# pkuyzy/TLC-GNN

Hardware: AMD Instinct MI355X
Metric: persistence-images/sec + LP-forward edges/sec, PubMed-scale, 1/2/4/8 GPU (higher is better)
Workload: dtype f64; 1 GPU

## Files before the change

### tlc-gnn_amd/csrc/pd_tiny.hip

```cpp
#include "tlc_common.h"
#include "tlc_kernels.h"

namespace {

template <typename T>
struct LaneArr {
    T* base;
    __device__ __forceinline__ T& operator[](int k) const { return base[k * 64]; }
};

struct LaneBytes8 {
    unsigned char* base;
    __device__ __forceinline__ unsigned char& operator[](int j) const { return base[(j >> 3) * 512 + (j & 7)]; }
};
struct LaneBytes8Slice {
    LaneBytes8 b;
    int off;
    __device__ __forceinline__ unsigned char& operator[](int j) const { return b[off + j]; }
};

__device__ __forceinline__ double tiny_key_asc(double fa, double fb) {
    const double hi = fa > fb ? fa : fb, lo = fa < fb ? fa : fb;
    return hi + (lo + 1.0) * 1e-6;
}
__device__ __forceinline__ double tiny_key_desc(double fa, double fb) {
    const double hi = fa > fb ? fa : fb, lo = fa < fb ? fa : fb;
    return lo - (101.0 - hi) * 1e-6;
}

__device__ __forceinline__ double tiny_norm_cdf(double x) {
    const double z = x * 0.70710678118654752440;
    const double t = z * z;
    double a = 4.22140728880708822e-18;
    a = fma(a, t, -8.03273501241577328e-17);
    a = fma(a, t, 1.44832646435981379e-15);
    a = fma(a, t, -2.46682701026445706e-14);
    a = fma(a, t, 3.95542951645852569e-13);
    a = fma(a, t, -5.94779401363763541e-12);
    a = fma(a, t, 8.35070279514723971e-11);
    a = fma(a, t, -1.08922210371485731e-09);
    a = fma(a, t, 1.31225329638028058e-08);
    a = fma(a, t, -1.45038522231504685e-07);
    a = fma(a, t, 1.45891690009337058e-06);
    a = fma(a, t, -1.32275132275132281e-05);
    a = fma(a, t, 1.06837606837606838e-04);
    a = fma(a, t, -7.57575757575757575e-04);
    a = fma(a, t, 4.62962962962962937e-03);
    a = fma(a, t, -2.38095238095238082e-02);
    a = fma(a, t, 1.00000000000000006e-01);
    a = fma(a, t, -3.33333333333333315e-01);
    a = fma(a, t, 1.0);
    return fma(0.5 * 1.1283791670955126, z * a, 0.5);
}

struct TinyImage {
    double px[25];
    __device__ __forceinline__ void clear() {
#pragma unroll
        for (int k = 0; k < 25; ++k) px[k] = 0.0;
    }
    __device__ __forceinline__ void add(double b, double d) {
        const double pers = d - b;
        const double wgt = pers < 0.0 ? 0.0 : (pers > 1.0 ? 1.0 : pers);
        if (wgt == 0.0) return;
        const double step = ((1.0 + 0.2) - 0.0) / 6.0;
        double cb[6], cp[6];
#pragma unroll
        for (int g = 0; g < 6; ++g) {
            cb[g] = tiny_norm_cdf((double)g * step - b);
            cp[g] = tiny_norm_cdf((double)g * step - pers);
        }
#pragma unroll
        for (int i = 0; i < 5; ++i) {
            const double db = cb[i + 1] - cb[i];
#pragma unroll
            for (int j = 0; j < 5; ++j) px[i * 5 + j] += wgt * (db * (cp[j + 1] - cp[j]));
        }
    }
};

constexpr int TN = TLC_T_NMAX, TM = TLC_T_MMAX;
constexpr int TP = TLC_T_NMAX + TLC_T_MMAX;
constexpr size_t T_OA = 0;
constexpr size_t T_OB = T_OA + (size_t)TM * 64 * 8;
constexpr size_t T_OC = T_OB + (size_t)TN * 64 * 8;
constexpr size_t T_OD = T_OC + (size_t)TN * 64 * 8;
constexpr size_t T_OE = T_OD + (size_t)TM * 64 * 2;
constexpr size_t TINY_WG_BYTES = T_OE + 5 * (size_t)TN * 64;
static_assert(2 * TP + 2 * TN <= TN * 8, "points + tree tables alias the second distance array (8 bytes per lane and row)");
static_assert(2 * (size_t)TM * 64 + (size_t)TN * 64 <= 5 * (size_t)TN * 64, "order / components / Pos-Neg list alias the tight-successor tables");

}

__device__ __forceinline__ void tiny_slot(const TlcPdParams p, unsigned char* lds, int lane, int slot) {
    LaneArr<double> ew{(double*)(lds + T_OA) + lane};
    const LaneArr<double>& key = ew;
    LaneArr<double> du{(double*)(lds + T_OB) + lane};
    const LaneArr<double>& f = du;
    LaneArr<double> dv{(double*)(lds + T_OC) + lane};
    const LaneArr<double>& dist = dv;
    LaneBytes8 cbytes{lds + T_OC + 8 * (size_t)lane};
    LaneBytes8Slice ptb{cbytes, 0};
    LaneBytes8Slice ptd{cbytes, TP};
    LaneBytes8Slice par{cbytes, 2 * TP};
    LaneBytes8Slice pedge{cbytes, 2 * TP + TN};
    LaneArr<unsigned short> eab{(unsigned short*)(lds + T_OD) + lane};
    LaneArr<unsigned char> cntU{lds + T_OE + lane};
    LaneArr<unsigned char> nxtU{lds + T_OE + (size_t)TN * 64 + lane};
    LaneArr<unsigned char> cntV{lds + T_OE + 2 * (size_t)TN * 64 + lane};
    LaneArr<unsigned char> nxtV{lds + T_OE + 3 * (size_t)TN * 64 + lane};
    LaneArr<unsigned char> ambl{lds + T_OE + 4 * (size_t)TN * 64 + lane};
    LaneArr<unsigned char> ord{lds + T_OE + lane};
    LaneArr<unsigned char> comp{lds + T_OE + (size_t)TM * 64 + lane};
    LaneArr<unsigned char> pn{lds + T_OE + (size_t)TM * 64 + (size_t)TN * 64 + lane};
    int npts = 0;
    int i, n, m2 = 0, lu, lv, m = 0;
    const unsigned* adir = nullptr;
    const double* alw = nullptr;
    {
        if (p.tiny_bin_list) {
            int s = slot, b = 0;
            while (b < TLC_TINY_BINS - 1 && s >= ((p.tiny_bin_cnt[b] + 63) >> 6)) { s -= (p.tiny_bin_cnt[b] + 63) >> 6; ++b; }
            const int wi = s * 64 + lane;
            if (wi >= p.tiny_bin_cnt[b]) return;
            i = p.tiny_bin_list[(size_t)b * p.tiny_bin_stride + wi];
        } else {
            int tier_count = p.tier_count;
            if (p.tier_count_dev) { const int c = *p.tier_count_dev; tier_count = c < tier_count ? c : tier_count; }
            const int wi = slot * 64 + lane;
            if (wi >= tier_count) return;
            i = p.tier_list[wi];
        }
        n = p.hdr_n[i]; m2 = p.hdr_m2[i]; lu = p.hdr_lu[i]; lv = p.hdr_lv[i];
        adir = p.small_dir ? p.small_dir + (size_t)i * (2 * TLC_S_MMAX) : p.A_dir + p.edge_off[i];
        alw = p.small_dir ? p.small_lw + (size_t)i * (2 * TLC_S_MMAX) : p.A_lw + p.edge_off[i];
    }
    int status = TLC_ST_OK;
    TinyImage img;
    img.clear();
    unsigned long long* pc = p.phase_cycles;
    unsigned long long t_prev = pc ? clock64() : 0ull;
#define TINY_STAMP(k) do { if (pc) { const unsigned long long _t = clock64(); if (lane == 0) atomicAdd(&pc[(k)], _t - t_prev); t_prev = _t; } } while (0)
    {
        for (int j0 = 0; j0 < m2; j0 += 8) {
            unsigned ee[8];
            double wq[8];
#pragma unroll
            for (int q = 0; q < 8; ++q) {
                const bool in = j0 + q < m2;
                ee[q] = in ? adir[j0 + q] : 0u;
                wq[q] = in ? alw[j0 + q] : 0.0;
            }
#pragma unroll
            for (int q = 0; q < 8; ++q) {
                const unsigned a = ee[q] >> 16, b = ee[q] & 0xffffu;
                if (j0 + q < m2 && a < b && m < TM) { eab[m] = (unsigned short)((a << 8) | b); ew[m] = wq[q]; ++m; }
            }
        }
    }
    TINY_STAMP(0);
    const double INF = __longlong_as_double(0x7FF0000000000000ll);
    auto bellman_ford_from = [&](int s, const LaneArr<double>& d) {
        for (int y = 0; y < n; ++y) d[y] = INF;
        d[s] = 0.0;
        for (int round = 0; round <= n; ++round) {
            bool ch = false;
            for (int e = 0; e < m; ++e) {
                const unsigned ab = eab[e];
                const int a = (int)(ab >> 8), b = (int)(ab & 0xffu);
                const double w = ew[e];
                const double da = d[a], db = d[b];
                const double ca = da + w, cb = db + w;
                if (ca < db) { d[b] = ca; ch = true; }
                if (cb < da) { d[a] = cb; ch = true; }
            }
            if (!ch) break;
        }
    };
    const bool far = lu < 0;
    if (far) {
        bellman_ford_from(0, dist);
        for (int y = 0; y < n; ++y) if (dist[y] == INF) status = TLC_ST_DISCONNECTED;
        if (status == TLC_ST_OK && n == 1) status = TLC_ST_NO_TREE_EDGE;
    } else {
        bellman_ford_from(lu, du);
        for (int y = 0; y < n; ++y) if (du[y] == INF) status = TLC_ST_DISCONNECTED;
        if (status == TLC_ST_OK) {
            bellman_ford_from(lv, dv);
            double dmx = 0.0;
            for (int y = 0; y < n; ++y) { const double a = du[y], b = dv[y]; dmx = a > dmx ? a : dmx; dmx = b > dmx ? b : dmx; cntU[y] = 0; cntV[y] = 0; }
            const double tol = 1e-10 * (1.0 + dmx);
            for (int e = 0; e < m; ++e) {
                const unsigned ab = eab[e];
                const int a = (int)(ab >> 8), b = (int)(ab & 0xffu);
                const double w = ew[e];
                const double ua = du[a], ub = du[b], va = dv[a], vb = dv[b];
                if (a != lu && (w + ub) - ua <= tol) { cntU[a] = (unsigned char)(cntU[a] + 1); nxtU[a] = (unsigned char)e; }
                if (b != lu && (w + ua) - ub <= tol) { cntU[b] = (unsigned char)(cntU[b] + 1); nxtU[b] = (unsigned char)e; }
                if (a != lv && (w + vb) - va <= tol) { cntV[a] = (unsigned char)(cntV[a] + 1); nxtV[a] = (unsigned char)e; }
                if (b != lv && (w + va) - vb <= tol) { cntV[b] = (unsigned char)(cntV[b] + 1); nxtV[b] = (unsigned char)e; }
            }
            double mx = 0.0;
            int namb = 0;
            for (int x = 0; x < n; ++x) {
                double fr = 0.0;
                if (x != lu && x != lv) {
                    double d1 = 0.0, d2 = 0.0;
                    bool amb = false;
                    int a = x, steps = 0;
                    while (a != lu) {
                        if (cntU[a] != 1 || ++steps > n) { amb = true; break; }
                        const int e = nxtU[a];
                        const unsigned ab = eab[e];
                        d1 = d1 + ew[e];
                        a = ((int)(ab >> 8) == a) ? (int)(ab & 0xffu) : (int)(ab >> 8);
                    }
                    a = x; steps = 0;
                    while (!amb && a != lv) {
                        if (cntV[a] != 1 || ++steps > n) { amb = true; break; }
                        const int e = nxtV[a];
                        const unsigned ab = eab[e];
                        d2 = d2 + ew[e];
                        a = ((int)(ab >> 8) == a) ? (int)(ab & 0xffu) : (int)(ab >> 8);
                    }
                    if (amb) ambl[namb++] = (unsigned char)x;
                    fr = d1 + d2;
                }
                f[x] = fr;
            }
            for (int q = 0; q < namb; ++q) {
                const int x = ambl[q];
                bellman_ford_from(x, dist);
                f[x] = dist[lu] + dist[lv];
            }
            if (namb && p.stats) atomicAdd(&p.stats[0], (unsigned long long)namb);
            for (int x = 0; x < n; ++x) { const double v = f[x]; mx = v > mx ? v : mx; }
            TINY_STAMP(1);
            if (mx == 0.0) status = TLC_ST_ZERO_RANGE;
            else for (int x = 0; x < n; ++x) f[x] = f[x] / mx;
        }
        if (status == TLC_ST_OK) {
            for (int e = 0; e < m; ++e) { const unsigned ab = eab[e]; key[e] = tiny_key_asc(f[ab >> 8], f[ab & 0xffu]); }
            for (int e = 0; e < m; ++e) {
                const double k = key[e];
                int r = 0;
                for (int e2 = 0; e2 < m; ++e2) { const double k2 = key[e2]; r += (k2 < k || (k2 == k && e2 < e)) ? 1 : 0; }
                ord[r] = (unsigned char)e;
            }
            auto find = [&](int x) {
                int c = comp[x];
                while (x != c) { const int g = comp[c]; comp[x] = (unsigned char)g; x = g; c = comp[x]; }
                return x;
            };
            for (int y = 0; y < n; ++y) comp[y] = (unsigned char)y;
            int imin = 0, imax = 0;
            {
                double fmin = f[0], fmax = f[0];
                for (int y = 1; y < n; ++y) { const double v = f[y]; if (v < fmin) { fmin = v; imin = y; } if (v > fmax) { fmax = v; imax = y; } }
            }
            for (int t = 0; t < m; ++t) {
                const unsigned ab = eab[ord[t]];
                const int a = (int)(ab >> 8), b = (int)(ab & 0xffu);
                const int pu = find(a), pv = find(b);
                if (pu != pv) {
                    const int small = (f[pu] <= f[pv]) ? pu : pv, large = pu + pv - small;
                    const int max_node = (f[a] > f[b]) ? a : b;
                    if (f[large] < f[max_node]) { ptb[npts] = (unsigned char)large; ptd[npts] = (unsigned char)max_node; ++npts; }
                    comp[large] = (unsigned char)small;
                }
            }
            TINY_STAMP(2);
            ptb[npts] = (unsigned char)imin; ptd[npts] = (unsigned char)imax; ++npts;
            for (int e = 0; e < m; ++e) { const unsigned ab = eab[e]; key[e] = tiny_key_desc(f[ab >> 8], f[ab & 0xffu]); }
            for (int e = 0; e < m; ++e) {
                const double k = key[e];
                int r = 0;
                for (int e2 = 0; e2 < m; ++e2) { const double k2 = key[e2]; r += (k2 > k || (k2 == k && e2 < e)) ? 1 : 0; }
                ord[r] = (unsigned char)e;
            }
            for (int y = 0; y < n; ++y) comp[y] = (unsigned char)y;
            int npos = 0, nneg = 0;
            for (int t = 0; t < m; ++t) {
                const int e = ord[t];
                const unsigned ab = eab[e];
                const int pu = find((int)(ab >> 8)), pv = find((int)(ab & 0xffu));
                if (pu != pv) {
                    pn[TM - 1 - nneg++] = (unsigned char)e;
                    const int small = (f[pu] <= f[pv]) ? pu : pv, large = pu + pv - small;
                    comp[small] = (unsigned char)large;
                } else {
                    pn[npos++] = (unsigned char)e;
                }
            }
            TINY_STAMP(3);
            if (nneg == 0) status = TLC_ST_NO_TREE_EDGE;
            else if (npos > 0) {
                for (int y = 0; y < n; ++y) par[y] = 0xFFu;
                const int root = (int)(eab[pn[TM - 1]] >> 8);
                par[root] = (unsigned char)root;
                for (int round = 0; round < n; ++round) {
                    bool ch = false;
                    for (int t = 0; t < nneg; ++t) {
                        const int e = pn[TM - 1 - t];
                        const unsigned ab = eab[e];
                        const int a = (int)(ab >> 8), b = (int)(ab & 0xffu);
                        const unsigned pa = par[a], pb = par[b];
                        if (pa != 0xFFu && pb == 0xFFu) { par[b] = (unsigned char)a; pedge[b] = (unsigned char)e; ch = true; }
                        else if (pb != 0xFFu && pa == 0xFFu) { par[a] = (unsigned char)b; pedge[a] = (unsigned char)e; ch = true; }
                    }
                    if (!ch) break;
                }
                for (int e = 0; e < m; ++e) { const unsigned ab = eab[e]; key[e] = tiny_key_asc(f[ab >> 8], f[ab & 0xffu]); }
                for (int t = 0; t < npos; ++t) {
                    const int e = pn[t];
                    const unsigned ab = eab[e];
                    const int pnode = (int)(ab >> 8), q = (int)(ab & 0xffu);
                    if (par[pnode] == 0xFFu || par[q] == 0xFFu) continue;
                    unsigned mask = 0u;
                    for (int a = pnode; a != root; a = par[a]) mask |= 1u << a;
                    int meet = root;
                    for (int a = q; a != root; a = par[a]) if ((mask >> a) & 1u) { meet = a; break; }
                    int best = -1, side = 0;
                    double bv = 0.0;
                    for (int a = pnode; a != meet; a = par[a]) { const double v = key[pedge[a]]; if (best < 0 || v > bv) { best = a; bv = v; side = 0; } }
                    for (int a = q; a != meet; a = par[a]) { const double v = key[pedge[a]]; if (best < 0 || v > bv) { best = a; bv = v; side = 1; } }
                    if (best < 0) continue;
                    const unsigned lab = eab[pedge[best]];
                    const double fa = f[lab >> 8], fb = f[lab & 0xffu];
                    const double large_value = fa > fb ? fa : fb;
                    const double fp = f[pnode], fq = f[q];
                    const double low_value = fp < fq ? fp : fq;
                    if (large_value > low_value && npts < TP) {
                        ptb[npts] = (unsigned char)(fp < fq ? pnode : q);
                        ptd[npts] = (unsigned char)(fa > fb ? (lab >> 8) : (lab & 0xffu));
                        ++npts;
                    }
                    int node = side == 0 ? pnode : q, nodec = side == 0 ? q : pnode, e_in = e;
                    while (nodec != best) {
                        const int tp = par[node], te = pedge[node];
                        par[node] = (unsigned char)nodec; pedge[node] = (unsigned char)e_in;
                        nodec = node; node = tp; e_in = te;
                    }
                }
            }
        }
    }
    TINY_STAMP(4);
    if (status == TLC_ST_OK)
        for (int t = 0; t < npts; ++t) img.add(f[ptb[t]], f[ptd[t]]);
    TINY_STAMP(5);
    double* out = p.out_pi + (size_t)i * 25;
    if (status != TLC_ST_OK) img.clear();
#pragma unroll
    for (int k = 0; k < 25; ++k) out[k] = img.px[k];
    if (p.out_status) p.out_status[i] = (unsigned char)status;
    TINY_STAMP(6);
    if (pc && lane == 0) atomicAdd(&pc[14], 1ull);
#undef TINY_STAMP
}

__global__ __launch_bounds__(64) void tlc_pd_tiny_kernel(TlcPdParams p) {
    extern __shared__ __attribute__((aligned(16))) unsigned char lds_all[];
    tiny_slot(p, lds_all, (int)(threadIdx.x & 63), (int)blockIdx.x);
}

int tlc_launch_pd_tiny(const TlcPdParams& p, void* stream) {
    if (p.tier_count <= 0) return TLC_OK;
    const size_t lds = TINY_WG_BYTES;
    int grid = (p.tier_count + 63) / 64;
    if (p.tiny_bin_list) {
        grid = 0;
        for (int b = 0; b < TLC_TINY_BINS; ++b) grid += (p.tiny_bin_cnt[b] + 63) / 64;
        if (grid == 0) return TLC_OK;
    }
    if (lds > 64 * 1024)
        TLC_HIP_CHECK(hipFuncSetAttribute((const void*)tlc_pd_tiny_kernel, hipFuncAttributeMaxDynamicSharedMemorySize, (int)lds));
    hipLaunchKernelGGL(tlc_pd_tiny_kernel, dim3(grid), dim3(64), lds, (hipStream_t)stream, p);
    TLC_HIP_CHECK(hipGetLastError());
    return TLC_OK;
}

__global__ __launch_bounds__(1024) void tlc_tiny_sort_kernel(int count, const int* __restrict__ list, const int* __restrict__ hdr_n,
                                                            const int* __restrict__ hdr_m2, int* __restrict__ out, int shift) {
    __shared__ int hist[64], base[64];
    const int tid = (int)threadIdx.x;
    if (tid < 64) hist[tid] = 0;
    __syncthreads();
    for (int k = tid; k < count; k += 1024) {
        const int i = list[k];
        int key = (hdr_n[i] + (hdr_m2[i] >> 1)) >> shift;
        key = key < 0 ? 0 : (key > 63 ? 63 : key);
        atomicAdd(&hist[63 - key], 1);
    }
    __syncthreads();
    if (tid == 0) { int run = 0; for (int b = 0; b < 64; ++b) { base[b] = run; run += hist[b]; } }
    __syncthreads();
    for (int k = tid; k < count; k += 1024) {
        const int i = list[k];
        int key = (hdr_n[i] + (hdr_m2[i] >> 1)) >> shift;
        key = key < 0 ? 0 : (key > 63 ? 63 : key);
        out[atomicAdd(&base[63 - key], 1)] = i;
    }
}

int tlc_launch_tiny_sort(int count, const int* list, const int* hdr_n, const int* hdr_m2, int* out, void* stream, int shift) {
    if (count <= 0) return TLC_OK;
    hipLaunchKernelGGL(tlc_tiny_sort_kernel, dim3(1), dim3(1024), 0, (hipStream_t)stream, count, list, hdr_n, hdr_m2, out, shift);
    TLC_HIP_CHECK(hipGetLastError());
    return TLC_OK;
}
```

Baseline: 78.93 million persistence-images/sec.

## Split each tiny subgraph across a lane pair sharing edges and workloads

```diff
diff --git a/tlc-gnn_amd/csrc/pd_tiny.hip b/tlc-gnn_amd/csrc/pd_tiny.hip
--- a/tlc-gnn_amd/csrc/pd_tiny.hip
+++ b/tlc-gnn_amd/csrc/pd_tiny.hip
@@ -7,6 +7,11 @@
 struct LaneArr {
     T* base;
     __device__ __forceinline__ T& operator[](int k) const { return base[k * 64]; }
+};
+
+struct PairRows {
+    double* base;
+    __device__ __forceinline__ double& operator[](int e) const { return base[(e >> 1) * 64 + (e & 1)]; }
 };
 
 struct LaneBytes8 {
@@ -19,13 +24,14 @@
     __device__ __forceinline__ unsigned char& operator[](int j) const { return b[off + j]; }
 };
 
-__device__ __forceinline__ double tiny_key_asc(double fa, double fb) {
-    const double hi = fa > fb ? fa : fb, lo = fa < fb ? fa : fb;
-    return hi + (lo + 1.0) * 1e-6;
-}
-__device__ __forceinline__ double tiny_key_desc(double fa, double fb) {
-    const double hi = fa > fb ? fa : fb, lo = fa < fb ? fa : fb;
-    return lo - (101.0 - hi) * 1e-6;
+__device__ __forceinline__ int pair_swap(int v) { return __builtin_amdgcn_mov_dpp(v, 0xB1, 0xF, 0xF, true); }
+__device__ __forceinline__ double pair_swap(double v) {
+    return __hiloint2double(pair_swap(__double2hiint(v)), pair_swap(__double2loint(v)));
+}
+__device__ __forceinline__ void pair_sync() {
+    __builtin_amdgcn_fence(__ATOMIC_RELEASE, "wavefront");
+    __builtin_amdgcn_wave_barrier();
+    __builtin_amdgcn_fence(__ATOMIC_ACQUIRE, "wavefront");
 }
 
 __device__ __forceinline__ double tiny_norm_cdf(double x) {
@@ -54,65 +60,68 @@
 }
 
 struct TinyImage {
-    double px[25];
+    double px[13];
     __device__ __forceinline__ void clear() {
 #pragma unroll
-        for (int k = 0; k < 25; ++k) px[k] = 0.0;
-    }
-    __device__ __forceinline__ void add(double b, double d) {
+        for (int k = 0; k < 13; ++k) px[k] = 0.0;
+    }
+    __device__ __forceinline__ void add(double b, double d, int h) {
         const double pers = d - b;
         const double wgt = pers < 0.0 ? 0.0 : (pers > 1.0 ? 1.0 : pers);
         if (wgt == 0.0) return;
         const double step = ((1.0 + 0.2) - 0.0) / 6.0;
-        double cb[6], cp[6];
-#pragma unroll
-        for (int g = 0; g < 6; ++g) {
-            cb[g] = tiny_norm_cdf((double)g * step - b);
-            cp[g] = tiny_norm_cdf((double)g * step - pers);
-        }
-#pragma unroll
-        for (int i = 0; i < 5; ++i) {
-            const double db = cb[i + 1] - cb[i];
-#pragma unroll
-            for (int j = 0; j < 5; ++j) px[i * 5 + j] += wgt * (db * (cp[j + 1] - cp[j]));
-        }
+        const double at = h ? pers : b;
+        double c[6], mine[5], other[5];
+#pragma unroll
+        for (int g = 0; g < 6; ++g) c[g] = tiny_norm_cdf((double)g * step - at);
+#pragma unroll
+        for (int g = 0; g < 5; ++g) { mine[g] = c[g + 1] - c[g]; other[g] = pair_swap(mine[g]); }
+        double row[3], col[5];
+#pragma unroll
+        for (int r = 0; r < 3; ++r) row[r] = h ? other[4 - r] : mine[r];
+#pragma unroll
+        for (int q = 0; q < 5; ++q) col[q] = h ? mine[4 - q] : other[q];
+#pragma unroll
+        for (int s = 0; s < 13; ++s) px[s] += wgt * (row[s / 5] * col[s % 5]);
     }
 };
 
 constexpr int TN = TLC_T_NMAX, TM = TLC_T_MMAX;
 constexpr int TP = TLC_T_NMAX + TLC_T_MMAX;
-constexpr size_t T_OA = 0;
-constexpr size_t T_OB = T_OA + (size_t)TM * 64 * 8;
-constexpr size_t T_OC = T_OB + (size_t)TN * 64 * 8;
-constexpr size_t T_OD = T_OC + (size_t)TN * 64 * 8;
-constexpr size_t T_OE = T_OD + (size_t)TM * 64 * 2;
-constexpr size_t TINY_WG_BYTES = T_OE + 5 * (size_t)TN * 64;
-static_assert(2 * TP + 2 * TN <= TN * 8, "points + tree tables alias the second distance array (8 bytes per lane and row)");
-static_assert(2 * (size_t)TM * 64 + (size_t)TN * 64 <= 5 * (size_t)TN * 64, "order / components / Pos-Neg list alias the tight-successor tables");
+constexpr size_t T_OK = 0;
+constexpr size_t T_OF = T_OK + (size_t)TM * 64 * 8;
+constexpr size_t T_OD = T_OF + (size_t)TN * 64 * 8;
+constexpr size_t T_OE = T_OD + (size_t)TM * 32 * 2;
+constexpr size_t T_E_ROWS = 2 * (size_t)TM + TN > 3 * (size_t)TN ? 2 * (size_t)TM + TN : 3 * (size_t)TN;
+constexpr size_t TINY_WG_BYTES = T_OE + T_E_ROWS * 64;
+static_assert(2 * TP + 2 * TN <= TN * 8, "points + tree tables alias B's column of the distance rows (8 bytes per lane and row)");
+static_assert((TM + 1) / 2 <= TM, "the pair's weights alias the first rows of its two key columns");
+static_assert(TN <= 32 && TM <= 255 && TP <= 255, "32-bit path mask; u8 edge and point indices");
+static_assert(T_OF % 8 == 0 && T_OD % 8 == 0 && T_OE % 2 == 0, "alignment of the regions");
 
 }
 
 __device__ __forceinline__ void tiny_slot(const TlcPdParams p, unsigned char* lds, int lane, int slot) {
-    LaneArr<double> ew{(double*)(lds + T_OA) + lane};
-    const LaneArr<double>& key = ew;
-    LaneArr<double> du{(double*)(lds + T_OB) + lane};
-    const LaneArr<double>& f = du;
-    LaneArr<double> dv{(double*)(lds + T_OC) + lane};
-    const LaneArr<double>& dist = dv;
-    LaneBytes8 cbytes{lds + T_OC + 8 * (size_t)lane};
+    const int h = lane & 1;
+    const int pr = lane >> 1, colA = lane & ~1, colB = lane | 1;
+    PairRows ew{(double*)(lds + T_OK) + colA};
+    LaneArr<double> key{(double*)(lds + T_OK) + lane};
+    LaneArr<double> dm{(double*)(lds + T_OF) + lane};
+    LaneArr<double> f{(double*)(lds + T_OF) + colA};
+    LaneArr<double> dist{(double*)(lds + T_OF) + colB};
+    LaneBytes8 cbytes{lds + T_OF + 8 * (size_t)colB};
     LaneBytes8Slice ptb{cbytes, 0};
     LaneBytes8Slice ptd{cbytes, TP};
     LaneBytes8Slice par{cbytes, 2 * TP};
     LaneBytes8Slice pedge{cbytes, 2 * TP + TN};
-    LaneArr<unsigned short> eab{(unsigned short*)(lds + T_OD) + lane};
-    LaneArr<unsigned char> cntU{lds + T_OE + lane};
-    LaneArr<unsigned char> nxtU{lds + T_OE + (size_t)TN * 64 + lane};
-    LaneArr<unsigned char> cntV{lds + T_OE + 2 * (size_t)TN * 64 + lane};
-    LaneArr<unsigned char> nxtV{lds + T_OE + 3 * (size_t)TN * 64 + lane};
-    LaneArr<unsigned char> ambl{lds + T_OE + 4 * (size_t)TN * 64 + lane};
+    LaneArr<unsigned short> eab{(unsigned short*)(lds + T_OD) + pr};
+    auto edge = [&](int e) -> unsigned { return eab.base[e * 32]; };
+    LaneArr<unsigned char> cnt{lds + T_OE + lane};
+    LaneArr<unsigned char> nxt{lds + T_OE + (size_t)TN * 64 + lane};
+    LaneArr<unsigned char> ambl{lds + T_OE + 2 * (size_t)TN * 64 + colA};
     LaneArr<unsigned char> ord{lds + T_OE + lane};
     LaneArr<unsigned char> comp{lds + T_OE + (size_t)TM * 64 + lane};
-    LaneArr<unsigned char> pn{lds + T_OE + (size_t)TM * 64 + (size_t)TN * 64 + lane};
+    LaneArr<unsigned char> pn{lds + T_OE + ((size_t)TM + TN) * 64 + colB};
     int npts = 0;
     int i, n, m2 = 0, lu, lv, m = 0;
     const unsigned* adir = nullptr;
@@ -120,14 +129,14 @@
     {
         if (p.tiny_bin_list) {
             int s = slot, b = 0;
-            while (b < TLC_TINY_BINS - 1 && s >= ((p.tiny_bin_cnt[b] + 63) >> 6)) { s -= (p.tiny_bin_cnt[b] + 63) >> 6; ++b; }
-            const int wi = s * 64 + lane;
+            while (b < TLC_TINY_BINS - 1 && s >= ((p.tiny_bin_cnt[b] + 31) >> 5)) { s -= (p.tiny_bin_cnt[b] + 31) >> 5; ++b; }
+            const int wi = s * 32 + pr;
             if (wi >= p.tiny_bin_cnt[b]) return;
             i = p.tiny_bin_list[(size_t)b * p.tiny_bin_stride + wi];
         } else {
             int tier_count = p.tier_count;
             if (p.tier_count_dev) { const int c = *p.tier_count_dev; tier_count = c < tier_count ? c : tier_count; }
-            const int wi = slot * 64 + lane;
+            const int wi = slot * 32 + pr;
             if (wi >= tier_count) return;
             i = p.tier_list[wi];
         }
@@ -142,22 +151,37 @@
     unsigned long long t_prev = pc ? clock64() : 0ull;
 #define TINY_STAMP(k) do { if (pc) { const unsigned long long _t = clock64(); if (lane == 0) atomicAdd(&pc[(k)], _t - t_prev); t_prev = _t; } } while (0)
     {
-        for (int j0 = 0; j0 < m2; j0 += 8) {
+        const int half = (m2 + 1) >> 1;
+        const int j_lo = h ? half : 0, j_hi = h ? m2 : half;
+        int mine = 0;
+        for (int j0 = j_lo; j0 < j_hi; j0 += 16) {
+            unsigned ee[16];
+#pragma unroll
+            for (int q = 0; q < 16; ++q) ee[q] = j0 + q < j_hi ? adir[j0 + q] : 0u;
+#pragma unroll
+            for (int q = 0; q < 16; ++q) mine += (ee[q] >> 16) < (ee[q] & 0xffffu) ? 1 : 0;
+        }
+        const int theirs = pair_swap(mine);
+        int at = h ? theirs : 0;
+        m = mine + theirs;
+        m = m < TM ? m : TM;
+        for (int j0 = j_lo; j0 < j_hi; j0 += 8) {
             unsigned ee[8];
             double wq[8];
 #pragma unroll
             for (int q = 0; q < 8; ++q) {
-                const bool in = j0 + q < m2;
+                const bool in = j0 + q < j_hi;
                 ee[q] = in ? adir[j0 + q] : 0u;
                 wq[q] = in ? alw[j0 + q] : 0.0;
             }
 #pragma unroll
             for (int q = 0; q < 8; ++q) {
                 const unsigned a = ee[q] >> 16, b = ee[q] & 0xffffu;
-                if (j0 + q < m2 && a < b && m < TM) { eab[m] = (unsigned short)((a << 8) | b); ew[m] = wq[q]; ++m; }
-            }
-        }
-    }
+                if (a < b && at < TM) { eab.base[at * 32] = (unsigned short)((a << 8) | b); ew[at] = wq[q]; ++at; }
+            }
+        }
+    }
+    pair_sync();
     TINY_STAMP(0);
     const double INF = __longlong_as_double(0x7FF0000000000000ll);
     auto bellman_ford_from = [&](int s, const LaneArr<double>& d) {
@@ -166,7 +190,7 @@
         for (int round = 0; round <= n; ++round) {
             bool ch = false;
             for (int e = 0; e < m; ++e) {
-                const unsigned ab = eab[e];
+                const unsigned ab = edge(e);
                 const int a = (int)(ab >> 8), b = (int)(ab & 0xffu);
                 const double w = ew[e];
                 const double da = d[a], db = d[b];
@@ -179,68 +203,72 @@
     };
     const bool far = lu < 0;
     if (far) {
-        bellman_ford_from(0, dist);
-        for (int y = 0; y < n; ++y) if (dist[y] == INF) status = TLC_ST_DISCONNECTED;
+        bellman_ford_from(0, dm);
+        for (int y = 0; y < n; ++y) if (dm[y] == INF) status = TLC_ST_DISCONNECTED;
         if (status == TLC_ST_OK && n == 1) status = TLC_ST_NO_TREE_EDGE;
     } else {
-        bellman_ford_from(lu, du);
-        for (int y = 0; y < n; ++y) if (du[y] == INF) status = TLC_ST_DISCONNECTED;
+        const int root = h ? lv : lu;
+        bellman_ford_from(root, dm);
+        for (int y = 0; y < n; ++y) if (dm[y] == INF) status = TLC_ST_DISCONNECTED;
+        status |= pair_swap(status);
         if (status == TLC_ST_OK) {
-            bellman_ford_from(lv, dv);
             double dmx = 0.0;
-            for (int y = 0; y < n; ++y) { const double a = du[y], b = dv[y]; dmx = a > dmx ? a : dmx; dmx = b > dmx ? b : dmx; cntU[y] = 0; cntV[y] = 0; }
+            for (int y = 0; y < n; ++y) { const double a = dm[y]; dmx = a > dmx ? a : dmx; cnt[y] = 0; }
+            { const double o = pair_swap(dmx); dmx = o > dmx ? o : dmx; }
             const double tol = 1e-10 * (1.0 + dmx);
             for (int e = 0; e < m; ++e) {
-                const unsigned ab = eab[e];
+                const unsigned ab = edge(e);
                 const int a = (int)(ab >> 8), b = (int)(ab & 0xffu);
                 const double w = ew[e];
-                const double ua = du[a], ub = du[b], va = dv[a], vb = dv[b];
-                if (a != lu && (w + ub) - ua <= tol) { cntU[a] = (unsigned char)(cntU[a] + 1); nxtU[a] = (unsigned char)e; }
-                if (b != lu && (w + ua) - ub <= tol) { cntU[b] = (unsigned char)(cntU[b] + 1); nxtU[b] = (unsigned char)e; }
-                if (a != lv && (w + vb) - va <= tol) { cntV[a] = (unsigned char)(cntV[a] + 1); nxtV[a] = (unsigned char)e; }
-                if (b != lv && (w + va) - vb <= tol) { cntV[b] = (unsigned char)(cntV[b] + 1); nxtV[b] = (unsigned char)e; }
-            }
-            double mx = 0.0;
+                const double xa = dm[a], xb = dm[b];
+                if (a != root && (w + xb) - xa <= tol) { cnt[a] = (unsigned char)(cnt[a] + 1); nxt[a] = (unsigned char)e; }
+                if (b != root && (w + xa) - xb <= tol) { cnt[b] = (unsigned char)(cnt[b] + 1); nxt[b] = (unsigned char)e; }
+            }
+            pair_sync();
             int namb = 0;
             for (int x = 0; x < n; ++x) {
                 double fr = 0.0;
                 if (x != lu && x != lv) {
-                    double d1 = 0.0, d2 = 0.0;
-                    bool amb = false;
+                    double dsum = 0.0;
+                    int amb = 0;
                     int a = x, steps = 0;
-                    while (a != lu) {
-                        if (cntU[a] != 1 || ++steps > n) { amb = true; break; }
-                        const int e = nxtU[a];
-                        const unsigned ab = eab[e];
-                        d1 = d1 + ew[e];
+                    while (a != root) {
+                        if (cnt[a] != 1 || ++steps > n) { amb = 1; break; }
+                        const int e = nxt[a];
+                        const unsigned ab = edge(e);
+                        dsum = dsum + ew[e];
                         a = ((int)(ab >> 8) == a) ? (int)(ab & 0xffu) : (int)(ab >> 8);
                     }
-                    a = x; steps = 0;
-                    while (!amb && a != lv) {
-                        if (cntV[a] != 1 || ++steps > n) { amb = true; break; }
-                        const int e = nxtV[a];
-                        const unsigned ab = eab[e];
-                        d2 = d2 + ew[e];
-                        a = ((int)(ab >> 8) == a) ? (int)(ab & 0xffu) : (int)(ab >> 8);
-                    }
-                    if (amb) ambl[namb++] = (unsigned char)x;
+                    const double dother = pair_swap(dsum);
+                    const double d1 = h ? dother : dsum, d2 = h ? dsum : dother;
+                    amb |= pair_swap(amb);
+                    if (amb) { if (!h) ambl[namb] = (unsigned char)x; ++namb; }
                     fr = d1 + d2;
                 }
-                f[x] = fr;
-            }
-            for (int q = 0; q < namb; ++q) {
+                if (!h) f[x] = fr;
+            }
+            for (int q = 0; q < (h ? 0 : namb); ++q) {
                 const int x = ambl[q];
                 bellman_ford_from(x, dist);
                 f[x] = dist[lu] + dist[lv];
             }
-            if (namb && p.stats) atomicAdd(&p.stats[0], (unsigned long long)namb);
+            if (namb && !h && p.stats) atomicAdd(&p.stats[0], (unsigned long long)namb);
+            pair_sync();
+            double mx = 0.0;
             for (int x = 0; x < n; ++x) { const double v = f[x]; mx = v > mx ? v : mx; }
             TINY_STAMP(1);
             if (mx == 0.0) status = TLC_ST_ZERO_RANGE;
-            else for (int x = 0; x < n; ++x) f[x] = f[x] / mx;
+            else for (int x = h; x < n; x += 2) f[x] = f[x] / mx;
+            pair_sync();
         }
         if (status == TLC_ST_OK) {
-            for (int e = 0; e < m; ++e) { const unsigned ab = eab[e]; key[e] = tiny_key_asc(f[ab >> 8], f[ab & 0xffu]); }
+            for (int e = 0; e < m; ++e) {
+                const unsigned ab = edge(e);
+                const double fa = f[ab >> 8], fb = f[ab & 0xffu];
+                const double hi = fa > fb ? fa : fb, lo = fa < fb ? fa : fb;
+                const double ka = hi + (lo + 1.0) * 1e-6, kd = lo - (101.0 - hi) * 1e-6;
+                key[e] = h ? -kd : ka;
+            }
             for (int e = 0; e < m; ++e) {
                 const double k = key[e];
                 int r = 0;
@@ -253,56 +281,51 @@
                 return x;
             };
             for (int y = 0; y < n; ++y) comp[y] = (unsigned char)y;
-            int imin = 0, imax = 0;
+            int iext = 0;
             {
-                double fmin = f[0], fmax = f[0];
-                for (int y = 1; y < n; ++y) { const double v = f[y]; if (v < fmin) { fmin = v; imin = y; } if (v > fmax) { fmax = v; imax = y; } }
-            }
+                double best = h ? -f[0] : f[0];
+                for (int y = 1; y < n; ++y) { const double v0 = f[y]; const double v = h ? -v0 : v0; if (v < best) { best = v; iext = y; } }
+            }
+            TINY_STAMP(2);
+            int npos = 0, nneg = 0;
             for (int t = 0; t < m; ++t) {
-                const unsigned ab = eab[ord[t]];
+                const int e = ord[t];
+                const unsigned ab = edge(e);
                 const int a = (int)(ab >> 8), b = (int)(ab & 0xffu);
                 const int pu = find(a), pv = find(b);
                 if (pu != pv) {
                     const int small = (f[pu] <= f[pv]) ? pu : pv, large = pu + pv - small;
-                    const int max_node = (f[a] > f[b]) ? a : b;
-                    if (f[large] < f[max_node]) { ptb[npts] = (unsigned char)large; ptd[npts] = (unsigned char)max_node; ++npts; }
-                    comp[large] = (unsigned char)small;
+                    if (!h) {
+                        const int max_node = (f[a] > f[b]) ? a : b;
+                        if (f[large] < f[max_node]) { ptb[npts] = (unsigned char)large; ptd[npts] = (unsigned char)max_node; ++npts; }
+                    } else {
+                        pn[TM - 1 - nneg] = (unsigned char)e;
+                    }
+                    ++nneg;
+                    comp[h ? small : large] = (unsigned char)(h ? large : small);
+                } else {
+                    if (h) pn[npos] = (unsigned char)e;
+                    ++npos;
                 }
             }
-            TINY_STAMP(2);
-            ptb[npts] = (unsigned char)imin; ptd[npts] = (unsigned char)imax; ++npts;
-            for (int e = 0; e < m; ++e) { const unsigned ab = eab[e]; key[e] = tiny_key_desc(f[ab >> 8], f[ab & 0xffu]); }
-            for (int e = 0; e < m; ++e) {
-                const double k = key[e];
-                int r = 0;
-                for (int e2 = 0; e2 < m; ++e2) { const double k2 = key[e2]; r += (k2 > k || (k2 == k && e2 < e)) ? 1 : 0; }
-                ord[r] = (unsigned char)e;
-            }
-            for (int y = 0; y < n; ++y) comp[y] = (unsigned char)y;
-            int npos = 0, nneg = 0;
-            for (int t = 0; t < m; ++t) {
-                const int e = ord[t];
-                const unsigned ab = eab[e];
-                const int pu = find((int)(ab >> 8)), pv = find((int)(ab & 0xffu));
-                if (pu != pv) {
-                    pn[TM - 1 - nneg++] = (unsigned char)e;
-                    const int small = (f[pu] <= f[pv]) ? pu : pv, large = pu + pv - small;
-                    comp[small] = (unsigned char)large;
-                } else {
-                    pn[npos++] = (unsigned char)e;
-                }
-            }
+            {
+                const int imax = pair_swap(iext);
+                if (!h) { ptb[npts] = (unsigned char)iext; ptd[npts] = (unsigned char)imax; ++npts; }
+                const int on = pair_swap(nneg), op = pair_swap(npos);
+                if (!h) { nneg = on; npos = op; }
+            }
+            pair_sync();
             TINY_STAMP(3);
             if (nneg == 0) status = TLC_ST_NO_TREE_EDGE;
-            else if (npos > 0) {
+            else if (npos > 0 && !h) {
                 for (int y = 0; y < n; ++y) par[y] = 0xFFu;
-                const int root = (int)(eab[pn[TM - 1]] >> 8);
-                par[root] = (unsigned char)root;
+                const int troot = (int)(edge(pn[TM - 1]) >> 8);
+                par[troot] = (unsigned char)troot;
                 for (int round = 0; round < n; ++round) {
                     bool ch = false;
                     for (int t = 0; t < nneg; ++t) {
                         const int e = pn[TM - 1 - t];
-                        const unsigned ab = eab[e];
+                        const unsigned ab = edge(e);
                         const int a = (int)(ab >> 8), b = (int)(ab & 0xffu);
                         const unsigned pa = par[a], pb = par[b];
                         if (pa != 0xFFu && pb == 0xFFu) { par[b] = (unsigned char)a; pedge[b] = (unsigned char)e; ch = true; }
@@ -310,22 +333,21 @@
                     }
                     if (!ch) break;
                 }
-                for (int e = 0; e < m; ++e) { const unsigned ab = eab[e]; key[e] = tiny_key_asc(f[ab >> 8], f[ab & 0xffu]); }
                 for (int t = 0; t < npos; ++t) {
                     const int e = pn[t];
-                    const unsigned ab = eab[e];
+                    const unsigned ab = edge(e);
                     const int pnode = (int)(ab >> 8), q = (int)(ab & 0xffu);
                     if (par[pnode] == 0xFFu || par[q] == 0xFFu) continue;
                     unsigned mask = 0u;
-                    for (int a = pnode; a != root; a = par[a]) mask |= 1u << a;
-                    int meet = root;
-                    for (int a = q; a != root; a = par[a]) if ((mask >> a) & 1u) { meet = a; break; }
+                    for (int a = pnode; a != troot; a = par[a]) mask |= 1u << a;
+                    int meet = troot;
+                    for (int a = q; a != troot; a = par[a]) if ((mask >> a) & 1u) { meet = a; break; }
                     int best = -1, side = 0;
                     double bv = 0.0;
                     for (int a = pnode; a != meet; a = par[a]) { const double v = key[pedge[a]]; if (best < 0 || v > bv) { best = a; bv = v; side = 0; } }
                     for (int a = q; a != meet; a = par[a]) { const double v = key[pedge[a]]; if (best < 0 || v > bv) { best = a; bv = v; side = 1; } }
                     if (best < 0) continue;
-                    const unsigned lab = eab[pedge[best]];
+                    const unsigned lab = edge(pedge[best]);
                     const double fa = f[lab >> 8], fb = f[lab & 0xffu];
                     const double large_value = fa > fb ? fa : fb;
                     const double fp = f[pnode], fq = f[q];
@@ -345,15 +367,18 @@
             }
         }
     }
+    pair_sync();
     TINY_STAMP(4);
+    npts += pair_swap(npts);
     if (status == TLC_ST_OK)
-        for (int t = 0; t < npts; ++t) img.add(f[ptb[t]], f[ptd[t]]);
+        for (int t = 0; t < npts; ++t) img.add(f[ptb[t]], f[ptd[t]], h);
     TINY_STAMP(5);
     double* out = p.out_pi + (size_t)i * 25;
     if (status != TLC_ST_OK) img.clear();
 #pragma unroll
-    for (int k = 0; k < 25; ++k) out[k] = img.px[k];
-    if (p.out_status) p.out_status[i] = (unsigned char)status;
+    for (int k = 0; k < 13; ++k)
+        if (k < 12 || !h) out[h ? 24 - k : k] = img.px[k];
+    if (p.out_status && !h) p.out_status[i] = (unsigned char)status;
     TINY_STAMP(6);
     if (pc && lane == 0) atomicAdd(&pc[14], 1ull);
 #undef TINY_STAMP
@@ -367,10 +392,10 @@
 int tlc_launch_pd_tiny(const TlcPdParams& p, void* stream) {
     if (p.tier_count <= 0) return TLC_OK;
     const size_t lds = TINY_WG_BYTES;
-    int grid = (p.tier_count + 63) / 64;
+    int grid = (p.tier_count + 31) / 32;
     if (p.tiny_bin_list) {
         grid = 0;
-        for (int b = 0; b < TLC_TINY_BINS; ++b) grid += (p.tiny_bin_cnt[b] + 63) / 64;
+        for (int b = 0; b < TLC_TINY_BINS; ++b) grid += (p.tiny_bin_cnt[b] + 31) / 32;
         if (grid == 0) return TLC_OK;
     }
     if (lds > 64 * 1024)
```

Result: no change. 79.15 million persistence-images/sec, median of 5 (+0.3%).
